# TritonDataCenter/node-zkstream

Measured on AMD Instinct MI355X. Metric: ZK ops/sec (whole node) + p50 get() RTT, 1M-znode synthetic tree, higher is better.
Workload: dtype uint8

## Files before the change

csrc/kernels/frame_scan.hip:

```cpp
#include "zk_frame_scan.h"

namespace zk {

__global__ __launch_bounds__(256) void fs_rows(
    const uint8_t* __restrict__ buf, const int64_t* __restrict__ n_dev,
    int64_t n_cap, const uint16_t* __restrict__ list,
    const uint16_t* __restrict__ pre, const int64_t* __restrict__ rec_meta,
    const int64_t* __restrict__ rec_entry,
    const int64_t* __restrict__ rec_exit,
    const int64_t* __restrict__ base, const int64_t* __restrict__ bsum,
    const int64_t* __restrict__ lastk, int64_t* __restrict__ foff,
    int32_t* __restrict__ flen, int64_t cap, uint64_t* __restrict__ lbw,
    uint64_t* __restrict__ lbw_tail) {
  __shared__ __attribute__((aligned(16))) uint8_t stage[4][FT_STAGE];
  const int lane = threadIdx.x & 63;
  const int wv = __builtin_amdgcn_readfirstlane((int)(threadIdx.x >> 6));
  const int64_t t = (int64_t)blockIdx.x * 4 + wv;
  const int64_t n = stream_len(n_dev, n_cap);
  if (t == 0) {
    if (lane == 0) {
      lbw_tail[LW_MINS] = 0;
      lbw_tail[LW_MINS + 1] = 0;
      lbw_tail[LW_NOSPEC] = 0;
      lbw_tail[LW_GRID + FL_NB] = 0;
    }
    if (lane < LW_END - LW_BIG) lbw_tail[LW_BIG + lane] = 0;
  }
  if (t * FT_S >= n) return;
  if (lane == 0) {
    lbw[2 * t] = 0;
    lbw[2 * t + 1] = 0;
  }
  if (t > *lastk) return;
  const int64_t b = bsum[t / FK_T] + base[t];
  const int64_t m = rec_meta[t];
  const int64_t x = rec_exit[t];
  const int32_t cnt = m_cnt(m);
  auto row = [&](int32_t k, int64_t p, int64_t q) {
    const int64_t idx = b + k;
    if (idx < cap) {
      foff[idx] = p + 4;
      flen[idx] = (int32_t)(q - p - 4);
    }
  };
  if (m_stale(m)) {
    const int32_t c = __builtin_amdgcn_readfirstlane(
        (int32_t)(rec_entry[t] - t * FT_S));
    fr_walk_stale<false>(buf, n, t, c, cnt, x, stage[wv], lane, row);
    return;
  }
  for (int32_t k = lane; k < cnt; k += 64) {
    int64_t p, q;
    fr_bounds(list, pre, t, m, x, k, p, q);
    row(k, p, q);
  }
}

__global__ __launch_bounds__(64) void fs_small(
    const uint8_t* __restrict__ buf, const int64_t* __restrict__ n_dev,
    int64_t n_cap, int64_t maxp, int64_t* __restrict__ foff,
    int32_t* __restrict__ flen, int64_t cap, int64_t* __restrict__ result) {
  __shared__ __attribute__((aligned(16))) uint8_t sb[FT_STAGE];
  const int lane = threadIdx.x;
  const int64_t n = stream_len(n_dev, n_cap);
  fc_stage<FT_S>(buf, n, 0, sb, lane);
  int32_t c = 0, k = 0;
  bool bad = false;
  const int32_t n32 = (int32_t)n;
  while (c + 4 <= n32) {
    const int32_t len = __builtin_amdgcn_readfirstlane(lds_be32(sb, c));
    if (len < 0 || (int64_t)len > maxp) { bad = true; break; }
    if (c + 4 + len > n32) break;
    if (lane == 0 && k < cap) {
      foff[k] = c + 4;
      flen[k] = len;
    }
    ++k;
    c += 4 + len;
  }
  if (lane == 0) {
    result[0] = k;
    result[1] = c;
    result[2] = bad ? 1 : 0;
    result[3] = k > cap ? 1 : 0;
  }
}

constexpr int32_t FS_LONG = 2;
constexpr int32_t FS_DEFER = 1 << 24;

constexpr int32_t FS_WIN_LONG = 1 << 16;

static int fs_window(int32_t window) {
  window &= FS_WIN_LONG - 1;
  return window <= 256 ? 256 : window <= 512 ? 512
       : window <= 1024 ? 1024 : 2048;
}

static int64_t* g_dbg = nullptr;
static int64_t g_dbg_tiles = 0;
static int64_t* fs_dbg_buf(int64_t tiles) {
  static int on = -1;
  if (on < 0) on = getenv("ZKMI_FS_DBG") != nullptr;
  if (!on) return nullptr;
  if (tiles > g_dbg_tiles) {
    if (g_dbg) (void)hipFree(g_dbg);
    if (hipMalloc(&g_dbg, (tiles + FL_DBG_ROWS) * 8 * 8) != hipSuccess)
      return nullptr;
    (void)hipMemset(g_dbg, 0, (tiles + FL_DBG_ROWS) * 8 * 8);
    g_dbg_tiles = tiles;
  }
  return g_dbg;
}

}

extern "C" {

int64_t zk_frame_scan_workspace(int64_t n) {
  return (int64_t)zk::fs_view(nullptr, n).total;
}

int zk_frame_scan(const uint8_t* buf, const int64_t* n_dev, int64_t n_cap,
                  int64_t maxp, uint8_t* ws, int64_t ws_bytes, int64_t* foff,
                  int32_t* flen, int64_t cap, int64_t* result, int32_t window,
                  int32_t clean, int32_t flags, hipStream_t st) {
  using namespace zk;
  const int W = fs_window(window);
  const bool defer = (flags & FS_DEFER) != 0;
  flags &= ~FS_DEFER;
  if (window & FS_WIN_LONG) flags |= FS_LONG;
  if (maxp > FC_MAXP || maxp < 0) return -3;
  const FsWs v = fs_view(ws, n_cap);
  if ((int64_t)v.total > ws_bytes) return -1;
  const int64_t tiles = v.tiles;
  if (defer && n_cap <= FT_S) return -5;
  if (n_cap <= FT_S && !(flags & (1 | 0xFFFF00)) &&
      fs_dbg_buf(tiles) == nullptr) {
    fs_small<<<1, 64, 0, st>>>(buf, n_dev, n_cap, maxp, foff, flen, cap,
                               result);
    ZK_LAUNCH_CHECK();
    return 0;
  }
  if (!clean && hipMemsetAsync(v.lbw, 0, v.lbw_bytes, st) != hipSuccess)
    return -4;
  int64_t* dbg = fs_dbg_buf(tiles);
  int G = ((flags >> 4) & 15) + 1;
  if ((flags & (FS_LONG | 1 | 0xFFFF00)) || W > 512) G = 1;
  G = G >= 8 ? 8 : G >= 4 ? 4 : G >= 2 ? 2 : 1;
  const TileLaunch tl{buf, n_dev, n_cap, maxp, &v, dbg, flags, W, G,
                      (flags & FS_LONG) != 0};
  int rc = G == 1 ? tile_launch(tl, st)
           : W == 256 ? group256_launch(tl, st) : group512_launch(tl, st);
  if (rc) return rc;
  rc = link_launch(buf, n_dev, n_cap, maxp, v, cap, result,
                   dbg ? dbg + 8 * tiles : nullptr, st);
  if (rc || defer) return rc;
  fs_rows<<<(unsigned)((tiles + 3) / 4), 256, 0, st>>>(
      buf, n_dev, n_cap, v.list, v.pre, v.rmeta, v.rent, v.rexit, v.base,
      v.bsum, &v.tail->lastk, foff, flen, cap, v.lbw, (uint64_t*)v.tail);
  ZK_LAUNCH_CHECK();
  return 0;
}

int zk_frame_tiles(const uint8_t* buf, const int64_t* n_dev, int64_t n_cap,
                   uint8_t* ws, int64_t ws_bytes, ZkFrameTiles* out) {
  using namespace zk;
  if (n_cap <= FT_S) return -2;
  const FsWs v = fs_view(ws, n_cap);
  if ((int64_t)v.total > ws_bytes) return -1;
  out->buf = buf;
  out->n_dev = n_dev;
  out->n_cap = n_cap;
  out->list = v.list;
  out->pre = v.pre;
  out->rec_meta = v.rmeta;
  out->rec_entry = v.rent;
  out->rec_exit = v.rexit;
  out->base = v.base;
  out->bsum = v.bsum;
  out->lastk = &v.tail->lastk;
  out->fblk = v.fblk;
  out->lbw = v.lbw;
  out->tiles = v.tiles;
  return 0;
}

int zk_frame_scan_stats(const uint8_t* ws, int64_t n_cap, uint32_t* out4,
                        hipStream_t st) {
  using namespace zk;
  FsTail* t = fs_view(const_cast<uint8_t*>(ws), n_cap).tail;
  const uint64_t* word[4] = {&t->nospec_total, &t->walked, &t->rounds,
                             &t->looked};
  for (int k = 0; k < 4; ++k)
    if (hipMemcpyAsync(out4 + k, word[k], 4, hipMemcpyDeviceToHost, st) !=
        hipSuccess)
      return -1;
  if (hipStreamSynchronize(st) != hipSuccess) return -1;
  if (hipMemsetAsync(t, 0, offsetof(FsTail, mins), st) != hipSuccess)
    return -1;
  return hipStreamSynchronize(st) == hipSuccess ? 0 : -1;
}

int zk_frame_scan_dbg(int64_t* host, int64_t tiles) {
  if (!zk::g_dbg || tiles > zk::g_dbg_tiles + zk::FL_DBG_ROWS) return -1;
  return hipMemcpy(host, zk::g_dbg, tiles * 8 * 8, hipMemcpyDeviceToHost) ==
                 hipSuccess ? 0 : -1;
}

}
```

csrc/kernels/zk_frame_tile.h:

```cpp
#pragma once
#include "zk_frame_scan.h"

namespace zk {

constexpr int FT_BITS = FT_S / 32;
constexpr int FT_XW = 2048 / 32;

ZK_DEV void ft_record(uint16_t* L, int32_t& m, uint32_t& ent, int32_t c,
                      int lane) {
  ent = lane == (m & 63) ? (uint32_t)c : ent;
  ++m;
  if ((m & 63) == 0) L[m - 64 + lane] = (uint16_t)ent;
}

ZK_DEV int32_t ft_starts_below(const uint32_t* sbits, int32_t c, int lane) {
  static_assert(FT_BITS == 2 * 64, "two map words per lane");
  const int32_t cw = c >> 5;
  int32_t below = 0;
#pragma unroll
  for (int h = 0; h < 2; ++h) {
    const int32_t wi = lane + 64 * h;
    const uint32_t wd = sbits[wi];
    below += wi < cw ? __popc(wd)
                     : (wi == cw ? __popc(wd & ((1u << (c & 31)) - 1u)) : 0);
  }
#pragma unroll
  for (int d = 32; d >= 1; d >>= 1) below += __shfl_xor(below, d, 64);
  return below;
}

ZK_DEV int64_t ft_cand(const uint8_t* sb, const uint32_t* sbits, int32_t e,
                       int32_t nrel, int32_t maxp, int64_t send, int64_t n,
                       int64_t ts, int32_t m, int lane) {
  int32_t c = e;
  int32_t hops = 0;
  for (;;) {
    if (c >= FT_S) return (ts + c) | ((int64_t)hops << CX_SHIFT);
    if (ts + c >= n) return FC_LIVE;
    const uint32_t smw = sbits[c >> 5];
    const int32_t lraw = lds_be32(sb, c);
    if ((smw >> (c & 31)) & 1u) {
      if (send & TERM) return (send & TBAD) ? FC_DEAD : FC_LIVE;
      const int32_t below = ft_starts_below(sbits, c, lane);
      return send | ((int64_t)(hops + m - below) << CX_SHIFT);
    }
    if (c + 4 > nrel) return FC_LIVE;
    const int32_t len = __builtin_amdgcn_readfirstlane(lraw);
    if ((uint32_t)len > (uint32_t)maxp) return FC_DEAD;
    const int32_t nx = c + 4 + len;
    if (nx > nrel) return FC_LIVE;
    ++hops;
    c = nx;
  }
}

constexpr int FT_NMAX = 512;
constexpr int FT_SLOTS = 352;
constexpr int32_t FT_LIMIT = FT_S;
enum : uint32_t {
  RK_NODE = 0, RK_EXIT = 1, RK_END = 2, RK_PART = 3, RK_BAD = 4, RK_SHORT = 5
};
ZK_DEV uint32_t rk(uint32_t kind, uint32_t val, uint32_t cnt) {
  return kind << 29 | val << 16 | cnt;
}
ZK_DEV uint32_t rk_kind(uint32_t w) { return w >> 29; }
ZK_DEV uint32_t rk_val(uint32_t w) { return (w >> 16) & 0x1FFF; }
ZK_DEV uint32_t rk_cnt(uint32_t w) { return w & 0xFFFF; }

constexpr int FT_SLOT_B = 704;
constexpr int FT_O_BLK = FT_STAGE;
constexpr int FT_O_BASE = FT_O_BLK + 64 * 8;
constexpr int FT_O_PK = FT_O_BASE + 64 * 2;
constexpr int FT_O_R = FT_O_PK + FT_NMAX * 4;
constexpr int FT_R_B = FT_NMAX * 2 > FT_SLOT_B + FT_XW * 4
                           ? FT_NMAX * 2 : FT_SLOT_B + FT_XW * 4;
constexpr int FT_O_XB = FT_O_R + FT_SLOT_B;
constexpr int FT_LDS = FT_O_R + FT_R_B;
static_assert(FT_SLOT_B >= FT_SLOTS * 2 && FT_SLOT_B >= FT_BITS * 4, "slots");
static_assert(FT_STAGE % 16 == 0 && FT_LDS % 16 == 0, "LDS alignment");

ZK_DEV int32_t be32_of(uint32_t lo, uint32_t hi, int32_t p) {
  return (int32_t)bswap32(__builtin_amdgcn_alignbyte(hi, lo, p & 3));
}

struct FtBlk {
  const uint64_t* mask;
  const uint16_t* base;
};

ZK_DEV bool ft_node(const FtBlk& blk, int32_t q, int32_t& idx) {
  const uint64_t m = blk.mask[q >> 6];
  const int32_t b = blk.base[q >> 6];
  const uint64_t bit = 1ull << (q & 63);
  idx = b + __popcll(m & (bit - 1));
  return (m & bit) != 0;
}

ZK_DEV uint32_t ft_classify(int32_t q, int32_t len, int32_t nrel,
                            int32_t maxp, int32_t minb, uint32_t before) {
  if (q + 4 > nrel) return rk(RK_PART, q, before);
  if ((uint32_t)len > (uint32_t)maxp) return rk(RK_BAD, q, before);
  const int32_t nx = q + 4 + len;
  if (nx > nrel) return rk(RK_PART, q, before);
  if (len < minb) return rk(RK_SHORT, q, before);
  if (nx >= FT_S) return rk(RK_EXIT, q, before + 1);
  return nx == nrel ? rk(RK_END, q, before + 1) : rk(RK_SHORT, q, before);
}

ZK_DEV uint32_t ft_root_at(const uint8_t* sb, const FtBlk& blk,
                           const uint32_t* pk, int32_t e, int32_t nrel,
                           int32_t maxp, int32_t minb) {
  int32_t j;
  if (ft_node(blk, e, j)) return pk[j];
  return ft_classify(e, lds_be32(sb, e), nrel, maxp, minb, 0);
}

ZK_DEV int32_t ft_next(const uint8_t* sb, int32_t p) {
  return p + 4 + lds_be32(sb, p);
}

ZK_DEV int64_t ft_cx(const uint8_t* sb, uint32_t w, int64_t ts) {
  switch (rk_kind(w)) {
    case RK_EXIT:
      return (ts + ft_next(sb, (int32_t)rk_val(w))) |
             ((int64_t)rk_cnt(w) << CX_SHIFT);
    case RK_BAD: return FC_DEAD;
    default: return FC_LIVE;
  }
}

ZK_DEV int64_t ft_send(const uint8_t* sb, uint32_t w, int64_t ts) {
  const int32_t v = (int32_t)rk_val(w);
  switch (rk_kind(w)) {
    case RK_EXIT: return ts + ft_next(sb, v);
    case RK_END: return TERM | (ts + ft_next(sb, v));
    case RK_BAD: return TERM | TBAD | (ts + v);
    default: return TERM | (ts + v);
  }
}

template <int NK>
struct FtNodes {
  int32_t p[NK];
  uint32_t w[NK];
};

template <int NK>
ZK_DEV int ft_build(FtNodes<NK>& me, const uint8_t* sb, const FtBlk& blk,
                    uint32_t* pk, const uint16_t* pos, int32_t N,
                    int32_t nrel, int32_t maxp, int32_t minb, int lane) {
#pragma unroll
  for (int k = 0; k < NK; ++k) {
    const int32_t i = lane + 64 * k;
    const int32_t p = pos[i < N ? i : 0];
// ... 120 lines not shown

template <int W>
ZK_DEV int32_t ft_cands_walk(const uint8_t* sb, const FtBlk& blk,
                             uint32_t* xbits, int32_t nrel, int32_t maxp,
                             int32_t& sx, int lane) {
  uint64_t best = 0;
  for (int r = 0; r < 2; ++r) {
    int32_t want = lane + 64 * r, p = -1;
    for (int b = 0; b < W / 64 && p < 0; ++b) {
      uint64_t m = blk.mask[b];
      const int32_t c = __popcll(m);
      if (want < c) {
        for (int k = 0; k < want; ++k) m &= m - 1;
        p = b * 64 + (int32_t)__builtin_ctzll(m);
      } else {
        want -= c;
      }
    }
    if (!__ballot(p >= 0)) break;
    int32_t c = p, cnt = 0, x = -1;
    bool live = p >= 0;
    while (live) {
      if (c + 4 > nrel) break;
      const int32_t len = lds_be32(sb, c);
      if ((uint32_t)len > (uint32_t)maxp) break;
      const int32_t nx = c + 4 + len;
      if (nx > nrel) break;
      ++cnt;
      if (nx >= FT_S) { x = nx - FT_S; break; }
      c = nx;
    }
    if (x >= 0) {
      if (x < W)
        __hip_atomic_fetch_or(&xbits[x >> 5], 1u << (x & 31),
                              __ATOMIC_RELAXED, __HIP_MEMORY_SCOPE_WAVEFRONT);
      const uint64_t key = (uint64_t)((uint32_t)cnt << 16 |
                                      (uint32_t)(0xFFFF - p)) << 32 |
                           (uint32_t)x;
      best = best > key ? best : key;
    }
  }
#pragma unroll
  for (int s = 32; s >= 1; s >>= 1) {
    const uint64_t o = (uint64_t)__shfl_xor((long long)best, s, 64);
    best = best > o ? best : o;
  }
  if (!best) return -1;
  sx = (int32_t)(uint32_t)best;
  return 0xFFFF - (int32_t)((best >> 32) & 0xFFFF);
}

template <int NK>
ZK_DEV int32_t ft_chain(const FtNodes<NK>& me, const uint8_t* sb,
                        const FtBlk& blk, uint16_t* slot, int32_t e,
                        uint32_t w, int lane) {
  const uint32_t kind = rk_kind(w);
  const int32_t D = (int32_t)rk_cnt(w);
  if (kind == RK_SHORT || kind == RK_BAD || D > FT_SLOTS) return -1;
  if (D == 0) return 0;
  const uint32_t root = w >> 16;
  int32_t hits = 0;
  bool on[NK];
#pragma unroll
  for (int k = 0; k < NK; ++k) {
    const int32_t c = (int32_t)rk_cnt(me.w[k]);
    const int32_t p = me.p[k];
    on[k] = p >= e && (me.w[k] >> 16) == root && c >= 1 && c <= D;
    if (on[k]) slot[D - c] = (uint16_t)p;
    hits += __popcll(__ballot(on[k]));
  }
  __builtin_amdgcn_wave_barrier();
  int32_t want = D;
  if (lane == 0) {
    slot[0] = (uint16_t)e;
    if (kind == RK_EXIT || kind == RK_END) slot[D - 1] = (uint16_t)rk_val(w);
  }
  if (kind == RK_EXIT || kind == RK_END) {
    int32_t j;
    if (!ft_node(blk, (int32_t)rk_val(w), j)) --want;
  }
  __builtin_amdgcn_wave_barrier();
  if (hits == want) return D;
  auto linked = [&]() {
    bool ok = true;
    for (int32_t k = lane; k < D; k += 64) {
      const int32_t p = slot[k];
      const int32_t nx = ft_next(sb, p);
      if (k + 1 < D) {
        ok &= nx == (int32_t)slot[k + 1];
      } else if (kind == RK_PART) {
        ok &= nx == (int32_t)rk_val(w);
      }
    }
    return __ballot(!ok) == 0;
  };
  if (linked()) return D;
  for (int it = 0; it < 8; ++it) {
    int32_t cur[NK];
#pragma unroll
    for (int k = 0; k < NK; ++k)
      cur[k] = on[k] ? (int32_t)slot[D - (int32_t)rk_cnt(me.w[k])] : 0;
    bool wr = false;
#pragma unroll
    for (int k = 0; k < NK; ++k) {
      if (on[k] && me.p[k] < cur[k]) {
        slot[D - (int32_t)rk_cnt(me.w[k])] = (uint16_t)me.p[k];
        wr = true;
      }
    }
    __builtin_amdgcn_wave_barrier();
    if (!__ballot(wr)) break;
  }
  return linked() ? D : -1;
}


struct FtTileRegs {
  uint4 v[FT_S / 16 / 64];
  uint4 pad;
};
ZK_DEV void ft_load(const uint8_t* __restrict__ buf, int64_t n, int64_t ts,
                    int lane, FtTileRegs& r) {
  constexpr int PER = FT_S / 16 / 64;
  r.pad = make_uint4(0, 0, 0, 0);
  if (ts + FT_STAGE <= n) {
#pragma unroll
    for (int j = 0; j < PER; ++j)
      __builtin_memcpy(&r.v[j], buf + ts + 16 * (lane + 64 * j), 16);
    if (lane == 0) __builtin_memcpy(&r.pad, buf + ts + FT_S, 16);
  } else {
#pragma unroll
    for (int j = 0; j < PER; ++j) {
      uint8_t* b = (uint8_t*)&r.v[j];
      const int64_t g = ts + 16 * (lane + 64 * j);
      for (int k = 0; k < 16; ++k) b[k] = g + k < n ? buf[g + k] : 0;
    }
    if (lane == 0) {
      uint8_t* b = (uint8_t*)&r.pad;
      for (int k = 0; k < 16; ++k)
        b[k] = ts + FT_S + k < n ? buf[ts + FT_S + k] : 0;
    }
  }
}
ZK_DEV void ft_store(uint8_t* sb, const FtTileRegs& r, int lane) {
  constexpr int PER = FT_S / 16 / 64;
#pragma unroll
  for (int j = 0; j < PER; ++j) *(uint4*)(sb + 16 * (lane + 64 * j)) = r.v[j];
  if (lane == 0) *(uint4*)(sb + FT_S) = r.pad;
  __builtin_amdgcn_wave_barrier();
}

ZK_DEV int64_t ft_walk(const uint8_t* sb, int32_t c, int32_t nrel,
                       int32_t maxp32, int64_t ts, uint16_t* L, int32_t& mo,
                       int lane) {
  int32_t m = 0, pb = 0;
  uint32_t ent = 0;
  int64_t send;
  c = __builtin_amdgcn_readfirstlane(c);
  nrel = __builtin_amdgcn_readfirstlane(nrel);
  const int32_t lim = min((int32_t)FT_S, nrel);
  if (c >= nrel) {
    send = TERM | (ts + c);
  } else {
    int32_t len = 0, nx = 0, last = 0;
    bool ok = true, fin = false;
    while (!fin) {
      len = __builtin_amdgcn_readfirstlane(lds_be32(sb, c));
      nx = c + 4 + len;
      ok = (uint32_t)len <= (uint32_t)maxp32 && nx <= nrel;
      if (!ok) break;
      ent = lane == (m & 63) ? (uint32_t)c : ent;
      ++m;
      if ((m & 63) == 0) {
        const int32_t q = m - 64 + lane;
        if (q >= pb) L[q] = (uint16_t)ent;
        pb = m;
      }
      if (nx >= lim) break;
      c = nx;
      if (4 + len != last) {
        last = 4 + len;
        continue;
      }
      const int32_t st = last;
      for (;;) {
        const int64_t s64 = (int64_t)c + (int64_t)lane * st;
        const int32_t sp = s64 < lim ? (int32_t)s64 : lim;
        const int32_t lv = sp < lim ? lds_be32(sb, sp) : -1;
        const bool acc = sp < lim && lv == st - 4 && sp + st <= nrel;
        const uint64_t no = ~__ballot(acc);
        const int32_t a = no ? (int32_t)__builtin_ctzll(no) : 64;
        if (a == 0) break;
        const uint64_t end = __ballot(acc && sp + st >= lim);
        const int32_t f = end ? (int32_t)__builtin_ctzll(end) : 64;
        const int32_t r = min(a, f + 1);
        const int32_t q = (m & ~63) + lane;
        if (q >= pb && q < m) L[q] = (uint16_t)ent;
        if (lane < r) L[m + lane] = (uint16_t)sp;
        m += r;
        pb = m;
        nx = c + r * st;
        len = st - 4;
        if (nx >= lim) {
          fin = true;
          break;
        }
        c = nx;
      }
    }
    if (!ok) {
      const bool bad = (c + 4 <= nrel) && ((len < 0) | (len > maxp32));
      send = TERM | (bad ? TBAD : 0) | (ts + c);
    } else if (nx >= FT_S) {
      send = ts + nx;
    } else {
      send = TERM | (ts + nx);
    }
  }
  {
    const int32_t q = (m & ~63) + lane;
    if (q >= pb && q < m) L[q] = (uint16_t)ent;
  }
  mo = m;
  return send;
}

ZK_DEV uint64_t ft_wait_prev(const uint64_t* lbw, int64_t t) {
  uint64_t x;
  int nap = 0;
  const uint64_t t_w = wall_clock64();
  for (;;) {
    x = lb_load(&lbw[2 * (t - 1)]);
    if (x != 0) break;
    if (wall_clock64() - t_w > FT_WAIT_TICKS) break;
    if (nap < 16) __builtin_amdgcn_s_sleep(2);
    else if (nap < 32) __builtin_amdgcn_s_sleep(8);
    else __builtin_amdgcn_s_sleep(32);
    ++nap;
  }
  return x;
}

ZK_DEV int64_t ft_pick(int64_t ts, bool has, int32_t e, int64_t xe,
                       uint32_t we, bool open, uint32_t& wE, bool& known) {
  const uint64_t hm = __ballot(has);
  const uint64_t lm = __ballot(has && xe != FC_DEAD);
  if (lm) {
    const int l = (int)__builtin_ctzll(lm);
    wE = (uint32_t)__builtin_amdgcn_readlane((int)we, l);
    known = !__builtin_amdgcn_readlane((int)open, l);
    return ts + __builtin_amdgcn_readlane(e, l);
  }
  return hm ? ts + __builtin_amdgcn_readlane(e, (int)__builtin_ctzll(hm)) : -1;
}

template <typename At>
ZK_DEV void ft_survivor_bits(uint32_t* sbits, int32_t m, int lane, At at) {
  for (int k = lane; k < FT_SLOT_B / 4; k += 64) sbits[k] = 0u;
  __builtin_amdgcn_wave_barrier();
  for (int i = lane; i < m; i += 64) {
    const uint32_t q = at(i);
    __hip_atomic_fetch_or(&sbits[q >> 5], 1u << (q & 31), __ATOMIC_RELAXED,
                          __HIP_MEMORY_SCOPE_WAVEFRONT);
  }
  __builtin_amdgcn_wave_barrier();
}

struct FtCtx {
  const uint8_t* buf;
  uint16_t* list;
  uint16_t* pre;
  int64_t* sx;
  uint64_t* lbw;
  int64_t* rec_entry;
  int64_t* rec_exit;
  int64_t* rec_meta;
  int32_t* rcount;
  int64_t* dbg;
  int64_t* cx;
  uint64_t* stats;
  uint8_t* sb;
  FtBlk blk;
  uint32_t* pk;
  uint16_t* pos;
  uint16_t* slot;
  uint32_t* sbits;
  uint32_t* xbits;
  int64_t n, t, ts, tend, t_0, t_s, t_d;
  int32_t nrel, maxp32, minb, N, misspec;
  bool nospec;
  int lane;
};

ZK_DEV void ft_join(const FtCtx& C, int64_t E, int32_t m, int64_t send,
                    FcWalk& wk) {
  const int lane = C.lane;
  const uint8_t* sb = C.sb;
  const int64_t n = C.n, ts = C.ts;
  const int32_t nrel = C.nrel, maxp32 = C.maxp32;
  int64_t c = E;
  uint16_t* P = C.pre + C.t * FT_LMAX;
  int32_t np = 0;
  uint32_t ent = 0;
  for (;;) {
    if (c >= C.tend) { wk.exit = c; break; }
    if (c >= n) { wk.exit = n; break; }
    const int32_t crel = (int32_t)(c - ts);
    const uint32_t smw = C.sbits[crel >> 5];
    const int32_t lraw = lds_be32(sb, crel);
    if ((smw >> (crel & 31)) & 1u) {
      wk.js = ft_starts_below(C.sbits, crel, lane);
      break;
    }
    const int32_t len = __builtin_amdgcn_readfirstlane(lraw);
    const int32_t nx = crel + 4 + len;
    if ((uint32_t)len > (uint32_t)maxp32 || nx > nrel) {
      wk.exit = c;
      wk.term = true;
      wk.bad = (crel + 4 <= nrel) && ((len < 0) | (len > maxp32));
      break;
    }
    ft_record(P, np, ent, crel, lane);
    c = ts + nx;
  }
  if (lane < (np & 63)) P[(np & ~63) + lane] = (uint16_t)ent;
  wk.np = np;
  wk.cnt = np;
  if (wk.js >= 0) {
    wk.cnt = np + (m - wk.js);
    fc_join_end(wk, send, n);
  }
}

ZK_DEV void ft_put_record(const FtCtx& C, int64_t t, int64_t send, int32_t m,
                          int64_t entry, const FcWalk& wk) {
  if (C.lane != 0) return;
  C.sx[t] = send;
  C.rcount[t] = m;
  C.rec_entry[t] = entry;
  C.rec_exit[t] = wk.exit;
  C.rec_meta[t] = fc_meta(wk);
}

ZK_DEV void ft_put_mapped(const FtCtx& C, int64_t send, int32_t m,
                          int64_t entry, const FcWalk& wk, int64_t t_1,
                          int64_t t_2, int64_t t_f, int rounds, bool done) {
  ft_put_record(C, C.t, send, m, entry, wk);
  if (C.lane == 0 && C.dbg) {
    int64_t* d = C.dbg + 8 * C.t;
    d[0] = C.t_0;
    d[1] = t_1;
    d[2] = t_2;
    d[3] = wall_clock64();
    d[4] = C.t_d;
    d[5] = (int64_t)C.N | (int64_t)rounds << 16 | (int64_t)done << 24;
    d[6] = C.t_s;
    d[7] = t_f;
  }
}

template <int W, bool LONG, int NK>
ZK_DEV int64_t fs_tile_rest(const FtCtx& cx_, bool mapped) {
  const FtCtx& C = cx_;
  const int lane = C.lane;
  const uint8_t* sb = C.sb;
  const int64_t n = C.n, t = C.t, ts = C.ts, tend = C.tend;
  const int32_t nrel = C.nrel, maxp32 = C.maxp32, minb = C.minb;
  constexpr int XW = W / 32;
  FtNodes<NK> me;
  int rounds = 0;
  if (mapped)
    rounds = ft_build<NK>(me, sb, C.blk, C.pk, C.pos, C.N, nrel, maxp32, minb,
                          lane);
  for (int k = lane; k < FT_R_B / 4; k += 64) C.sbits[k] = 0u;
  __builtin_amdgcn_wave_barrier();
  const int64_t t_f = C.dbg ? wall_clock64() : 0;

  int32_t px = -1, sp = -1;
  {
    int32_t x = -1;
    sp = mapped ? ft_cands<W, LONG, NK>(me, sb, C.xbits, x)
                : ft_cands_walk<W>(sb, C.blk, C.xbits, nrel, maxp32, x, lane);
    if (sp >= 0 && x >= 0 && x < (LONG ? FT_S - 1 : W)) px = x;
  }
  __builtin_amdgcn_wave_barrier();
  uint64_t word = (uint64_t)1 << 63;
  if (px >= 0) word |= (uint64_t)(px + 1);
  {
    uint32_t xw = lane < XW ? C.xbits[lane] : 0u;
    if (px >= 0 && px < W && lane == (px >> 5)) xw &= ~(1u << (px & 31));
    uint64_t any = __ballot(xw != 0);
    int nsl = 1;
    if (px < 0 && any) {
      const int wl = (int)__builtin_ctzll(any);
      const uint32_t bits = (uint32_t)__builtin_amdgcn_readlane((int)xw, wl);
      const int x0 = wl * 32 + (int)__builtin_ctz(bits);
      word |= (uint64_t)(x0 + 1);
      if (lane == wl) xw &= ~(1u << (x0 & 31));
      any = __ballot(xw != 0);
    }
    while (any && nsl < 5) {
      const int wl = (int)__builtin_ctzll(any);
      uint32_t bits = (uint32_t)__builtin_amdgcn_readlane((int)xw, wl);
      while (bits && nsl < 5) {
        const int bit = (int)__builtin_ctz(bits);
        bits &= bits - 1;
        word |= (uint64_t)(wl * 32 + bit + 1) << (12 * nsl);
        ++nsl;
      }
      any &= any - 1;
    }
  }
  if (lane == 0) lb_store(&C.lbw[2 * t], word);
  const int64_t t_1 = C.dbg ? wall_clock64() : 0;

  int64_t E = 0;
  bool none = false;
  uint32_t wE = 0;
  bool wE_ok = false;
  if (t > 0 && C.nospec) {
    none = true;
    if (lane < 5) C.cx[5 * t + lane] = FC_DEAD;
  } else if (t > 0) {
    const uint64_t x = ft_wait_prev(C.lbw, t);
    const int32_t v = lane < 5 ? (int32_t)((x >> (12 * lane)) & 0xFFF) : 0;
    const bool has = v != 0 && ts + (v - 1) < n;
    const int32_t e = v - 1;
    uint32_t we = 0;
    if (has && mapped) we = ft_root_at(sb, C.blk, C.pk, e, nrel, maxp32, minb);
    const bool open = has && (!mapped || rk_kind(we) == RK_SHORT);
    int64_t xe = has && !open ? ft_cx(sb, we, ts) : FC_DEAD;
    for (uint64_t um = __ballot(open); um; um &= um - 1) {
      const int l = (int)__builtin_ctzll(um);
      const int32_t el = __builtin_amdgcn_readlane(e, l);
      const int64_t r = ft_cand(sb, C.sbits, el, nrel, maxp32, -1, n, ts, 0,
                                lane);
      if (lane == l) xe = r;
    }
    if (lane < 5) C.cx[5 * t + lane] = xe;
    E = ft_pick(ts, has, e, xe, we, open, wE, wE_ok);
    wE_ok = wE_ok && mapped;
    if (C.misspec > 0 && t % C.misspec == 1 && E >= 0 && E + 1 < n) {
      ++E;
      wE_ok = false;
    }
    none = E < 0;
  }
  const int64_t t_2 = C.dbg ? wall_clock64() : 0;

  uint16_t* L = C.list + t * FT_LMAX;
  FcWalk wk{E, 0, 0, -1, false, false};
  int64_t send = -1;
  int32_t m = 0;
  bool done = false;
  const int32_t erel = (int32_t)(E - ts);
  if (!none && erel >= nrel) {
    send = TERM | E;
    fc_join_end(wk, send, n);
    done = true;
  } else if (!none && mapped) {
    const uint32_t we = wE_ok ? wE
                              : ft_root_at(sb, C.blk, C.pk, erel, nrel, maxp32,
                                           minb);
    const int32_t D = ft_chain<NK>(me, sb, C.blk, C.slot, erel, we, lane);
    if (D >= 0) {
      for (int32_t k = lane; k < D; k += 64) L[k] = C.slot[k];
      m = D;
      send = ft_send(sb, we, ts);
      wk.cnt = D;
      wk.js = D > 0 ? 0 : -1;
      fc_join_end(wk, send, n);
      done = true;
    }
  }
  if (!done) {
    if (sp >= 0 && mapped) {
      const uint32_t ws = ft_root_at(sb, C.blk, C.pk, sp, nrel, maxp32, minb);
      const int32_t D = ft_chain<NK>(me, sb, C.blk, C.slot, sp, ws, lane);
      if (D > 0) {
        for (int32_t k = lane; k < D; k += 64) L[k] = C.slot[k];
        m = D;
        send = ft_send(sb, ws, ts);
      }
    } else if (sp >= 0) {
      __builtin_amdgcn_wave_barrier();
      send = ft_walk(sb, sp, nrel, maxp32, ts, L, m, lane);
      if (m == 0) send = -1;
    }
    __builtin_amdgcn_wave_barrier();
    ft_survivor_bits(C.sbits, m, lane, [&](int i) { return (uint32_t)L[i]; });
    if (!none) {
      ft_join(C, E, m, send, wk);
    } else {
      if (m > 0) fc_join_end(wk, send, n);
      if (lane == 0) fc_stat(C.stats, 1, 1), fc_stat(C.stats, LW_NOSPEC, 1);
    }
  }
  ft_put_mapped(C, send, m, none ? -1 : E, wk, t_1, t_2, t_f, rounds, done);
  return send;
}


ZK_DEV int64_t ft_cx_of(int64_t send, int32_t m) {
  if (!(send & TERM)) return send | ((int64_t)m << CX_SHIFT);
  return (send & TBAD) ? FC_DEAD : FC_LIVE;
}

template <int SVN>
ZK_DEV int32_t ft_sv_at(const uint32_t (&sv)[SVN], int32_t q) {
  uint32_t v = 0;
#pragma unroll
  for (int i = 0; i < SVN; ++i)
    if (i == (q >> 6)) v = sv[i];
  return __builtin_amdgcn_readlane((int)v, q & 63);
}

template <int W, int G>
ZK_DEV void ft_group_tail(const FtCtx& C, int64_t send0, bool alive,
                          FtTileRegs& nxt) {
  const int lane = C.lane;
  uint8_t* sb = C.sb;
  const int64_t n = C.n, t0 = C.t;
  const int32_t maxp32 = C.maxp32;
  const int64_t ntiles = (n + FT_S - 1) / FT_S;
  int64_t send = send0;
  int32_t kdone = 1;
  for (int k = 1; k < G; ++k) {
    const int64_t tk = t0 + k;
    if (tk >= ntiles) break;
    const int64_t tsk = tk * FT_S;
    const int64_t c = send;
    const bool live = alive && !(send & TERM) && c >= tsk &&
                      c < tsk + FT_S;
    if (!live) break;
    int64_t* const dk = C.dbg ? C.dbg + 8 * tk : nullptr;
    const int64_t k_0 = dk ? wall_clock64() : 0;
    ft_store(sb, nxt, lane);
    const int64_t k_1 = dk ? wall_clock64() : 0;
    if (k + 1 < G && tk + 1 < ntiles) ft_load(C.buf, n, tsk + FT_S, lane, nxt);
    int32_t m;
    const int32_t nrelk = (int32_t)min(n - tsk, (int64_t)1 << 30);
    send = ft_walk(sb, (int32_t)(c - tsk), nrelk, maxp32, tsk,
                   C.list + tk * FT_LMAX, m, lane);
    const int64_t k_2 = dk ? wall_clock64() : 0;
    FcWalk wk{c, m, 0, m > 0 ? 0 : -1, false, false};
    fc_join_end(wk, send, n);
    ft_put_record(C, tk, send, m, c, wk);
    if (lane == 0) {
      lb_store(&C.lbw[2 * (tk - 1)],
               (uint64_t)1 << 63 | (uint64_t)(c - tsk + 1));
      C.cx[5 * tk] = ft_cx_of(send, m);
      if (dk) {
        dk[0] = k_0;
        dk[1] = k_1;
        dk[2] = k_2;
        dk[3] = wall_clock64();
        dk[5] = (int64_t)m;
      }
    }
    if (lane >= 1 && lane < 5) C.cx[5 * tk + lane] = FC_DEAD;
    kdone = k + 1;
  }
  for (int k = kdone; k < G; ++k) {
    const int64_t tk = t0 + k;
    if (tk >= ntiles) break;
    if (lane == 0) lb_store(&C.lbw[2 * (tk - 1)], (uint64_t)1 << 63);
    ft_put_record(C, tk, -1, 0, -1, FcWalk{-1, 0, 0, -1, false, false});
    if (lane < 5) C.cx[5 * tk + lane] = FC_DEAD;
  }
  const int64_t tl = min(t0 + G, ntiles) - 1;
  {
    uint64_t word = (uint64_t)1 << 63;
    const int64_t tle = (tl + 1) * FT_S;
    if (kdone == (int32_t)(tl - t0 + 1) && alive && !(send & TERM) &&
        send >= tle && send < tle + W)
      word |= (uint64_t)(send - tle + 1);
    if (lane == 0) lb_store(&C.lbw[2 * tl], word);
  }
}

template <int W, int NK, int G>
ZK_DEV void fs_group_rest(const FtCtx& cx_) {
  static_assert(G > 1 && W <= 512, "groups: small windows");
  constexpr int WJ = W / 64;
  const FtCtx& C = cx_;
  const int lane = C.lane;
  uint8_t* sb = C.sb;
  const int64_t n = C.n, t0 = C.t, ts = C.ts;
  const int32_t nrel = C.nrel, maxp32 = C.maxp32, minb = C.minb;
  const int64_t ntiles = (n + FT_S - 1) / FT_S;
  FtNodes<NK> me;
  const int rounds = ft_build<NK>(me, sb, C.blk, C.pk, C.pos, C.N, nrel,
                                  maxp32, minb, lane);
  for (int k = lane; k < FT_R_B / 4; k += 64) C.sbits[k] = 0u;
  __builtin_amdgcn_wave_barrier();
  const int64_t t_f = C.dbg ? wall_clock64() : 0;

  int32_t x = -1;
  const int32_t sp = ft_cands<W, false, NK>(me, sb, C.xbits, x);
  uint32_t rw[WJ];
  int64_t rx[WJ];
#pragma unroll
  for (int j = 0; j < WJ; ++j) {
    const int32_t e = lane + 64 * j;
    rw[j] = e < nrel ? ft_root_at(sb, C.blk, C.pk, e, nrel, maxp32, minb)
                     : rk(RK_END, 0, 0);
    rx[j] = e < nrel ? ft_cx(sb, rw[j], ts) : FC_LIVE;
  }
  int32_t m0 = 0;
  int64_t send0 = -1;
  uint32_t ws = 0;
  uint16_t* L0 = C.list + t0 * FT_LMAX;
  if (sp >= 0) {
    ws = ft_root_at(sb, C.blk, C.pk, sp, nrel, maxp32, minb);
    const int32_t D = ft_chain<NK>(me, sb, C.blk, C.slot, sp, ws, lane);
    if (D >= 0) {
      for (int32_t k = lane; k < D; k += 64) L0[k] = C.slot[k];
      m0 = D;
      send0 = ft_send(sb, ws, ts);
    } else {
      __builtin_amdgcn_wave_barrier();
      send0 = ft_walk(sb, sp, nrel, maxp32, ts, L0, m0, lane);
      for (int32_t k = lane; k < m0; k += 64) C.slot[k] = L0[k];
      ws = 0;
    }
  }
  constexpr int SVN = (FT_SLOTS + 63) / 64;
  __builtin_amdgcn_wave_barrier();
  uint32_t sv[SVN];
#pragma unroll
  for (int i = 0; i < SVN; ++i)
    sv[i] = lane + 64 * i < m0 ? C.slot[lane + 64 * i] : 0u;
  const int64_t t_1 = C.dbg ? wall_clock64() : 0;

  FtTileRegs nxt;
  if (G > 1 && t0 + 1 < ntiles) ft_load(C.buf, n, ts + FT_S, lane, nxt);
  ft_group_tail<W, G>(C, send0, sp >= 0, nxt);

  int64_t E = 0;
  bool none = false;
  uint32_t wE = 0;
  bool known = false;
  bool staged = false;
  auto restage = [&]() {
    if (staged) return;
    FtTileRegs r;
    ft_load(C.buf, n, ts, lane, r);
    ft_store(sb, r, lane);
    ft_survivor_bits(C.sbits, m0, lane, [&](int i) {
      uint32_t v = 0;
#pragma unroll
      for (int k = 0; k < SVN; ++k)
        if (k == (i >> 6)) v = sv[k];
      return v;
    });
    staged = true;
  };
  if (t0 > 0) {
    const uint64_t xw = ft_wait_prev(C.lbw, t0);
    const int32_t v = lane < 5 ? (int32_t)((xw >> (12 * lane)) & 0xFFF) : 0;
    const bool has = v != 0 && ts + (v - 1) < n;
    const int32_t e = v - 1;
    uint32_t we = 0;
    int64_t xe = FC_DEAD;
    bool open = false;
    for (int s = 0; s < 5; ++s) {
      const int32_t es = __builtin_amdgcn_readlane(e, s);
      if (!__builtin_amdgcn_readlane((int)has, s)) continue;
      if (es >= W) {
        if (lane == s) open = true;
        continue;
      }
      const int jj = es >> 6, ll = es & 63;
      uint32_t wv = 0;
      int64_t xv = 0;
#pragma unroll
      for (int j = 0; j < WJ; ++j)
        if (j == jj) { wv = rw[j]; xv = rx[j]; }
      const uint32_t wsv = (uint32_t)__builtin_amdgcn_readlane((int)wv, ll);
      const int64_t xsv = (int64_t)(
          (uint64_t)(uint32_t)__builtin_amdgcn_readlane((int)(uint32_t)xv,
                                                         ll) |
          (uint64_t)(uint32_t)__builtin_amdgcn_readlane(
              (int)(uint32_t)((uint64_t)xv >> 32), ll) << 32);
      if (lane == s) {
        we = wsv;
        xe = xsv;
        open = rk_kind(wsv) == RK_SHORT;
      }
    }
    if (__ballot(open)) {
      restage();
      for (uint64_t um = __ballot(open); um; um &= um - 1) {
        const int l = (int)__builtin_ctzll(um);
        const int32_t el = __builtin_amdgcn_readlane(e, l);
        const int64_t r = ft_cand(sb, C.sbits, el, nrel, maxp32, send0, n,
                                  ts, m0, lane);
        if (lane == l) xe = r;
      }
    }
    if (lane < 5) C.cx[5 * t0 + lane] = xe;
    E = ft_pick(ts, has, e, xe, we, open, wE, known);
    none = E < 0;
  } else {
    wE = rw[0];
    wE = (uint32_t)__builtin_amdgcn_readlane((int)wE, 0);
    known = true;
  }
  const int64_t t_2 = C.dbg ? wall_clock64() : 0;

  FcWalk wk{E, 0, 0, -1, false, false};
  const int32_t erel = (int32_t)(E - ts);
  bool done = false;
  if (!none && erel >= nrel) {
    fc_join_end(wk, TERM | E, n);
    done = true;
  } else if (!none && known && ws != 0 && (wE >> 16) == (ws >> 16) &&
             (int32_t)rk_cnt(wE) <= m0 && rk_cnt(wE) > 0 &&
             ft_sv_at<SVN>(sv, m0 - (int32_t)rk_cnt(wE)) == erel) {
    wk.js = m0 - (int32_t)rk_cnt(wE);
    wk.cnt = (int32_t)rk_cnt(wE);
    fc_join_end(wk, send0, n);
    done = true;
  }
  if (!done && !none) {
    restage();
    ft_join(C, E, m0, send0, wk);
  } else if (none) {
    if (m0 > 0) fc_join_end(wk, send0, n);
    if (lane == 0) fc_stat(C.stats, 1, 1), fc_stat(C.stats, LW_NOSPEC, 1);
  }
  ft_put_mapped(C, send0, m0, none ? -1 : E, wk, t_1, t_2, t_f, rounds, done);
}

template <int W, bool LONG, int G>
__global__ __launch_bounds__(256) void fs_tile(
    const uint8_t* __restrict__ buf, const int64_t* __restrict__ n_dev,
    int64_t n_cap, int64_t maxp, uint16_t* __restrict__ list,
    uint16_t* __restrict__ pre, int64_t* __restrict__ sx, uint64_t* lbw,
    int64_t* __restrict__ rec_entry, int64_t* __restrict__ rec_exit,
    int64_t* __restrict__ rec_meta, int32_t* __restrict__ rcount,
    int64_t ntiles_cap, int64_t* __restrict__ dbg, int32_t minb,
    int32_t tflags, int64_t* __restrict__ cx) {
  static_assert(W % 64 == 0 && W <= 2048, "window");
  extern __shared__ __attribute__((aligned(16))) uint8_t smem_all[];
  const int wv = __builtin_amdgcn_readfirstlane((int)(threadIdx.x >> 6));
  uint8_t* smem = smem_all + wv * FT_LDS;
  FtCtx C;
  C.sb = smem;
  uint64_t* bmask = (uint64_t*)(smem + FT_O_BLK);
  uint16_t* bbase = (uint16_t*)(smem + FT_O_BASE);
  C.blk.mask = bmask;
  C.blk.base = bbase;
  C.pk = (uint32_t*)(smem + FT_O_PK);
  C.pos = (uint16_t*)(smem + FT_O_R);
  C.slot = (uint16_t*)(smem + FT_O_R);
  C.sbits = (uint32_t*)(smem + FT_O_R);
  C.xbits = (uint32_t*)(smem + FT_O_XB);
  const int lane = threadIdx.x & 63;
  const int64_t n = stream_len(n_dev, n_cap);
  const int64_t ntiles = (n + FT_S - 1) / FT_S;
  const int64_t t = ((int64_t)blockIdx.x * (blockDim.x >> 6) + wv) * G;
  if (t >= ntiles) return;
  C.t_0 = dbg ? wall_clock64() : 0;
  const int64_t ts = t * FT_S;
  const int64_t tend = ts + FT_S;
  const int32_t nrel = (int32_t)min(n - ts, (int64_t)1 << 30);
  const int32_t maxp32 = (int32_t)maxp;
  uint8_t* sb = C.sb;

  {
    FtTileRegs r;
    ft_load(buf, n, ts, lane, r);
    ft_store(sb, r, lane);
  }
  C.t_s = dbg ? (__builtin_amdgcn_s_waitcnt(0), wall_clock64()) : 0;

  int32_t N;
  {
    const int32_t P0 = lane * 64;
    uint32_t d[17];
    {
      const int r = (lane >> 2) & 3;
      uint4 x0 = *(const uint4*)(sb + P0 + 16 * (r & 3));
      uint4 x1 = *(const uint4*)(sb + P0 + 16 * ((1 + r) & 3));
      uint4 x2 = *(const uint4*)(sb + P0 + 16 * ((2 + r) & 3));
      uint4 x3 = *(const uint4*)(sb + P0 + 16 * ((3 + r) & 3));
      const uint32_t pad = *(const uint32_t*)(sb + FT_S);
      auto sel = [](bool c, uint4 a, uint4 b) {
        return make_uint4(c ? a.x : b.x, c ? a.y : b.y, c ? a.z : b.z,
                          c ? a.w : b.w);
      };
      {
        const bool c = r & 1;
        const uint4 y0 = sel(c, x3, x0), y1 = sel(c, x0, x1),
                    y2 = sel(c, x1, x2), y3 = sel(c, x2, x3);
        x0 = y0; x1 = y1; x2 = y2; x3 = y3;
      }
      {
        const bool c = r & 2;
        const uint4 y0 = sel(c, x2, x0), y1 = sel(c, x3, x1),
                    y2 = sel(c, x0, x2), y3 = sel(c, x1, x3);
        x0 = y0; x1 = y1; x2 = y2; x3 = y3;
      }
      d[0] = x0.x; d[1] = x0.y; d[2] = x0.z; d[3] = x0.w;
      d[4] = x1.x; d[5] = x1.y; d[6] = x1.z; d[7] = x1.w;
      d[8] = x2.x; d[9] = x2.y; d[10] = x2.z; d[11] = x2.w;
      d[12] = x3.x; d[13] = x3.y; d[14] = x3.z; d[15] = x3.w;
      const uint32_t nx = (uint32_t)__shfl_down((int)d[0], 1, 64);
      d[16] = lane == 63 ? pad : nx;
    }
    const uint32_t lim = P0 < W ? (uint32_t)(maxp32 - minb + 1)
                         : LONG ? (uint32_t)(FT_LIMIT - minb)
                                : (uint32_t)(W - 3 - minb);
    uint32_t lo = 0, hi = 0;
#pragma unroll
    for (int j = 0; j < 32; ++j) {
      const uint32_t v = (uint32_t)be32_of(d[j >> 2], d[(j >> 2) + 1], j);
      lo |= ((v - (uint32_t)minb) < lim ? 1u : 0u) << j;
    }
#pragma unroll
    for (int j = 32; j < 64; ++j) {
      const uint32_t v = (uint32_t)be32_of(d[j >> 2], d[(j >> 2) + 1], j);
      hi |= ((v - (uint32_t)minb) < lim ? 1u : 0u) << (j - 32);
    }
    uint64_t mask = (uint64_t)hi << 32 | lo;
    const int32_t room = nrel - 4 - P0;
    if (room < 63) mask = room < 0 ? 0 : mask & ((2ull << room) - 1);
    const uint32_t c = (uint32_t)__popcll(mask);
    uint32_t incl = c;
#pragma unroll
    for (int s = 1; s < 64; s <<= 1) {
      const uint32_t y = __shfl_up(incl, s, 64);
      if (lane >= s) incl += y;
    }
    N = __builtin_amdgcn_readlane((int)incl, 63);
    const uint32_t base = incl - c;
    bmask[lane] = mask;
    bbase[lane] = (uint16_t)base;
    if (N <= FT_NMAX) {
      uint32_t k = base;
      uint64_t m = mask;
      while (m) {
        C.pos[k++] = (uint16_t)(P0 + __builtin_ctzll(m));
        m &= m - 1;
      }
    }
  }
  __builtin_amdgcn_wave_barrier();
  C.t_d = dbg ? wall_clock64() : 0;
  C.buf = buf; C.list = list; C.pre = pre; C.sx = sx; C.lbw = lbw;
  C.rec_entry = rec_entry; C.rec_exit = rec_exit; C.rec_meta = rec_meta;
  C.rcount = rcount; C.dbg = dbg; C.cx = cx;
  C.stats = &lbw[2 * ntiles_cap];
  C.n = n; C.t = t; C.ts = ts; C.tend = tend;
  C.nrel = nrel; C.maxp32 = maxp32; C.minb = minb; C.N = N;
  C.nospec = tflags & 1;
  C.misspec = tflags >> 8;
  C.lane = lane;
  static_assert(FT_NMAX == 512, "node buckets");
  if constexpr (G > 1) {
    static_assert(!LONG, "groups: frames within the window");
    if (N <= 128) fs_group_rest<W, 2, G>(C);
    else if (N <= 256) fs_group_rest<W, 4, G>(C);
    else if (N <= FT_NMAX) fs_group_rest<W, 8, G>(C);
    else {
      const int64_t s0 = fs_tile_rest<W, LONG, 1>(C, false);
      FtTileRegs nxt;
      if (t + 1 < (n + FT_S - 1) / FT_S) ft_load(buf, n, ts + FT_S, lane, nxt);
      ft_group_tail<W, G>(C, s0, s0 >= 0, nxt);
    }
  } else {
    if (N <= 128) fs_tile_rest<W, LONG, 2>(C, true);
    else if (N <= 256) fs_tile_rest<W, LONG, 4>(C, true);
    else if (N <= FT_NMAX) fs_tile_rest<W, LONG, 8>(C, true);
    else fs_tile_rest<W, LONG, 1>(C, false);
  }
}



template <int W, bool LONG, int G>
int fs_tile_launch(const TileLaunch& l, hipStream_t st) {
  const FsWs& w = *l.ws;
  const int64_t waves = (w.tiles + G - 1) / G;
  const unsigned blocks = (unsigned)((waves + FS_TPB - 1) / FS_TPB);
  fs_tile<W, LONG, G><<<blocks, 64 * FS_TPB, FT_LDS * FS_TPB, st>>>(
      l.buf, l.n_dev, l.n_cap, l.maxp, w.list, w.pre, w.sx, w.lbw, w.rent,
      w.rexit, w.rmeta, w.rcnt, w.tiles, l.dbg, FS_MINB, l.tflags, w.cx);
  ZK_LAUNCH_CHECK();
  return 0;
}

template <int W>
int fs_group_launch(const TileLaunch& l, hipStream_t st) {
  switch (l.G) {
    case 8: return fs_tile_launch<W, false, 8>(l, st);
    case 4: return fs_tile_launch<W, false, 4>(l, st);
    case 2: return fs_tile_launch<W, false, 2>(l, st);
    default: return -1;
  }
}

}
```

Baseline: 2.188 billion.

## Skip tiles in group tail by gathering fixed-stride frame runs in bulk

When the frames ending a tile form a run of equal length, the group tail now checks the whole strided run with one gathered global load per lane. It then writes records, list entries and link words for every tile the run covers, so those tiles skip the serial per-tile walk. The register survivor vector becomes a 16-bit LDS array, which saves registers. Group mode is also allowed when the debug, nospec and misspec flags are set, and the commit adds nospec and misspec test paths. The risk lies in correctness on edge cases such as runs crossing tiles and partial final frames.

After: 2.312 billion, median of 6. 1.06x the previous value.

```diff
diff --git a/csrc/kernels/frame_scan.hip b/csrc/kernels/frame_scan.hip
--- a/csrc/kernels/frame_scan.hip
+++ b/csrc/kernels/frame_scan.hip
@@ -146,7 +146,7 @@
     return -4;
   int64_t* dbg = fs_dbg_buf(tiles);
   int G = ((flags >> 4) & 15) + 1;
-  if ((flags & (FS_LONG | 1 | 0xFFFF00)) || W > 512) G = 1;
+  if ((flags & FS_LONG) || W > 512) G = 1;
   G = G >= 8 ? 8 : G >= 4 ? 4 : G >= 2 ? 2 : 1;
   const TileLaunch tl{buf, n_dev, n_cap, maxp, &v, dbg, flags, W, G,
                       (flags & FS_LONG) != 0};
diff --git a/csrc/kernels/zk_frame_tile.h b/csrc/kernels/zk_frame_tile.h
--- a/csrc/kernels/zk_frame_tile.h
+++ b/csrc/kernels/zk_frame_tile.h
@@ -1,5 +1,6 @@
 #pragma once
 #include "zk_frame_scan.h"
+#include "zk_run_span.h"
 
 namespace zk {
 
@@ -426,17 +427,19 @@
 
 ZK_DEV int64_t ft_walk(const uint8_t* sb, int32_t c, int32_t nrel,
                        int32_t maxp32, int64_t ts, uint16_t* L, int32_t& mo,
-                       int lane) {
+                       int lane, int32_t& last, bool& run) {
   int32_t m = 0, pb = 0;
   uint32_t ent = 0;
   int64_t send;
   c = __builtin_amdgcn_readfirstlane(c);
   nrel = __builtin_amdgcn_readfirstlane(nrel);
+  last = __builtin_amdgcn_readfirstlane(last);
+  run = false;
   const int32_t lim = min((int32_t)FT_S, nrel);
   if (c >= nrel) {
     send = TERM | (ts + c);
   } else {
-    int32_t len = 0, nx = 0, last = 0;
+    int32_t len = 0, nx = 0;
     bool ok = true, fin = false;
     while (!fin) {
       len = __builtin_amdgcn_readfirstlane(lds_be32(sb, c));
@@ -450,12 +453,18 @@
         if (q >= pb) L[q] = (uint16_t)ent;
         pb = m;
       }
-      if (nx >= lim) break;
+      if (nx >= lim) {
+        run = 4 + len == last;
+        last = 4 + len;
+        break;
+      }
       c = nx;
       if (4 + len != last) {
         last = 4 + len;
+        run = false;
         continue;
       }
+      run = true;
       const int32_t st = last;
       for (;;) {
         const int64_t s64 = (int64_t)c + (int64_t)lane * st;
@@ -606,14 +615,17 @@
   }
 }
 
-ZK_DEV void ft_put_record(const FtCtx& C, int64_t t, int64_t send, int32_t m,
-                          int64_t entry, const FcWalk& wk) {
-  if (C.lane != 0) return;
+ZK_DEV void ft_put_record_lane(const FtCtx& C, int64_t t, int64_t send,
+                               int32_t m, int64_t entry, const FcWalk& wk) {
   C.sx[t] = send;
   C.rcount[t] = m;
   C.rec_entry[t] = entry;
   C.rec_exit[t] = wk.exit;
   C.rec_meta[t] = fc_meta(wk);
+}
+ZK_DEV void ft_put_record(const FtCtx& C, int64_t t, int64_t send, int32_t m,
+                          int64_t entry, const FcWalk& wk) {
+  if (C.lane == 0) ft_put_record_lane(C, t, send, m, entry, wk);
 }
 
 ZK_DEV void ft_put_mapped(const FtCtx& C, int64_t send, int32_t m,
@@ -758,7 +770,9 @@
       }
     } else if (sp >= 0) {
       __builtin_amdgcn_wave_barrier();
-      send = ft_walk(sb, sp, nrel, maxp32, ts, L, m, lane);
+      int32_t last = 0;
+      bool run;
+      send = ft_walk(sb, sp, nrel, maxp32, ts, L, m, lane, last, run);
       if (m == 0) send = -1;
     }
     __builtin_amdgcn_wave_barrier();
@@ -780,26 +794,127 @@
   return (send & TBAD) ? FC_DEAD : FC_LIVE;
 }
 
-template <int SVN>
-ZK_DEV int32_t ft_sv_at(const uint32_t (&sv)[SVN], int32_t q) {
-  uint32_t v = 0;
-#pragma unroll
-  for (int i = 0; i < SVN; ++i)
-    if (i == (q >> 6)) v = sv[i];
-  return __builtin_amdgcn_readlane((int)v, q & 63);
+constexpr int FT_NGI = 4;
+static_assert(RUN_TILE == FT_S, "zk_run_span.h: the tile");
+struct FtGather {
+  uint32_t w[FT_NGI];
+  int32_t crel, S, room, want, nrel;
+  int64_t g_0;
+};
+ZK_DEV FtGather ft_gather_issue(const FtCtx& C, int64_t c, int32_t S,
+                                int64_t tk, int64_t gend) {
+  FtGather g;
+  const int64_t tsk = tk * FT_S;
+  g.crel = __builtin_amdgcn_readfirstlane((int32_t)(c - tsk));
+  g.S = __builtin_amdgcn_readfirstlane(S);
+  g.g_0 = C.dbg ? wall_clock64() : 0;
+  g.room = (int32_t)(gend - tk);
+  g.nrel = (int32_t)min(C.n - tsk, (int64_t)1 << 30);
+  g.want = run_want(g.crel, g.S, g.room * FT_S, 64 * FT_NGI);
+  const uint8_t* tb = C.buf + tsk;
+#pragma unroll
+  for (int i = 0; i < FT_NGI; ++i) {
+    const int32_t j = C.lane + 64 * i;
+    const int32_t prel = g.crel + j * g.S;
+    g.w[i] = 0;
+    if (j < g.want && run_word_in(prel, g.nrel))
+      __builtin_memcpy(&g.w[i], tb + prel, 4);
+  }
+  return g;
+}
+ZK_DEV int32_t ft_gather_take(const FtCtx& C, const FtGather& g, int64_t tk,
+                              int64_t& send, bool& full) {
+  const int lane = C.lane;
+  const int64_t n = C.n, tsk = tk * FT_S;
+  const int32_t crel = g.crel, S = g.S, want = g.want, room = g.room;
+  const uint32_t(&w)[FT_NGI] = g.w;
+  const int64_t g_0 = g.g_0;
+  const int64_t g_1 =
+      C.dbg ? (__builtin_amdgcn_s_waitcnt(0), wall_clock64()) : 0;
+  int32_t a = 0;
+  bool open = true;
+#pragma unroll
+  for (int i = 0; i < FT_NGI; ++i) {
+    const int32_t j = lane + 64 * i;
+    const int32_t prel = crel + j * S;
+    const bool acc = j < want && run_word_in(prel, g.nrel) &&
+                     run_accept((int32_t)bswap32(w[i]), S, prel, g.nrel,
+                                C.maxp32);
+    const uint64_t no = ~__ballot(acc);
+    const int32_t ai = no ? (int32_t)__builtin_ctzll(no) : 64;
+    a += open ? ai : 0;
+    open = open && ai == 64;
+  }
+  full = a == 64 * FT_NGI;
+  const int32_t cov = min(run_tiles_covered(crel, S, a), room);
+  if (cov == 0) return 0;
+  const int64_t g_2 = C.dbg ? wall_clock64() : 0;
+  int32_t rfirst = 0;
+  if (lane < cov) {
+    const RunTile r = run_tile(crel, S, a, lane);
+    rfirst = r.first;
+    const int64_t tq = tk + lane;
+    const int64_t entry = tsk + r.entry, exit = tsk + r.exit;
+    FcWalk wk{entry, r.count, 0, r.count > 0 ? 0 : -1, false, false};
+    fc_join_end(wk, exit, n);
+    ft_put_record_lane(C, tq, exit, r.count, entry, wk);
+    lb_store(&C.lbw[2 * (tq - 1)],
+             (uint64_t)1 << 63 | (uint64_t)(entry - tq * FT_S + 1));
+    C.cx[5 * tq] = ft_cx_of(exit, r.count);
+#pragma unroll
+    for (int s = 1; s < 5; ++s) C.cx[5 * tq + s] = FC_DEAD;
+    if (C.dbg) {
+      int64_t* const dk = C.dbg + 8 * tq;
+      dk[0] = g_0;
+      dk[1] = g_1;
+      dk[2] = g_2;
+      dk[3] = wall_clock64();
+      dk[5] = (int64_t)r.count;
+    }
+  }
+#pragma unroll
+  for (int i = 0; i < FT_NGI; ++i) {
+    const int32_t j = lane + 64 * i;
+    const int32_t prel = crel + j * S;
+    const int32_t q = prel >> 12;
+    const int32_t first = __shfl(rfirst, q & 63, 64);
+    if (j < a && q < cov) {
+      C.list[(tk + q) * FT_LMAX + (j - first)] = (uint16_t)(prel & (FT_S - 1));
+    }
+  }
+  send = tsk + run_tile(crel, S, a, cov - 1).exit;
+  return cov;
 }
 
 template <int W, int G>
 ZK_DEV void ft_group_tail(const FtCtx& C, int64_t send0, bool alive,
-                          FtTileRegs& nxt) {
+                          FtTileRegs& nxt, int32_t last, bool run) {
   const int lane = C.lane;
   uint8_t* sb = C.sb;
   const int64_t n = C.n, t0 = C.t;
   const int32_t maxp32 = C.maxp32;
   const int64_t ntiles = (n + FT_S - 1) / FT_S;
+  const int64_t gend = min(t0 + G, ntiles);
   int64_t send = send0;
   int32_t kdone = 1;
-  for (int k = 1; k < G; ++k) {
+  int k = 1;
+  if (W <= 256 && run && last >= 16 && last <= FT_S && t0 + 1 < ntiles &&
+      alive && !(send & TERM)) {
+    bool full = true, first = true;
+    while (full && k < G && t0 + k < ntiles && send >= (t0 + k) * FT_S &&
+           send < (t0 + k + 1) * FT_S) {
+      const FtGather g = ft_gather_issue(C, send, last, t0 + k, gend);
+      if (first) ft_store(sb, nxt, lane);
+      first = false;
+      const int32_t cov = ft_gather_take(C, g, t0 + k, send, full);
+      if (cov == 0) break;
+      k += cov;
+    }
+    kdone = k;
+    if (k < G && t0 + k < ntiles)
+      ft_load(C.buf, n, (t0 + k) * FT_S, lane, nxt);
+  }
+  for (; k < G; ++k) {
     const int64_t tk = t0 + k;
     if (tk >= ntiles) break;
     const int64_t tsk = tk * FT_S;
@@ -815,7 +930,7 @@
     int32_t m;
     const int32_t nrelk = (int32_t)min(n - tsk, (int64_t)1 << 30);
     send = ft_walk(sb, (int32_t)(c - tsk), nrelk, maxp32, tsk,
-                   C.list + tk * FT_LMAX, m, lane);
+                   C.list + tk * FT_LMAX, m, lane, last, run);
     const int64_t k_2 = dk ? wall_clock64() : 0;
     FcWalk wk{c, m, 0, m > 0 ? 0 : -1, false, false};
     fc_join_end(wk, send, n);
@@ -894,22 +1009,31 @@
       send0 = ft_send(sb, ws, ts);
     } else {
       __builtin_amdgcn_wave_barrier();
-      send0 = ft_walk(sb, sp, nrel, maxp32, ts, L0, m0, lane);
+      int32_t last = 0;
+      bool run;
+      send0 = ft_walk(sb, sp, nrel, maxp32, ts, L0, m0, lane, last, run);
       for (int32_t k = lane; k < m0; k += 64) C.slot[k] = L0[k];
       ws = 0;
     }
   }
-  constexpr int SVN = (FT_SLOTS + 63) / 64;
+  static_assert(FT_SLOTS * 2 <= FT_NMAX * 4, "the starts fit the node words");
   __builtin_amdgcn_wave_barrier();
-  uint32_t sv[SVN];
-#pragma unroll
-  for (int i = 0; i < SVN; ++i)
-    sv[i] = lane + 64 * i < m0 ? C.slot[lane + 64 * i] : 0u;
+  uint16_t* const sv = (uint16_t*)C.pk;
+  for (int32_t k = lane; k < m0; k += 64) sv[k] = C.slot[k];
+  __builtin_amdgcn_wave_barrier();
+  int32_t last0 = 0;
+  bool run0 = false;
+  if (m0 >= 1 && send0 >= 0 && !(send0 & TERM)) {
+    const int32_t a = __builtin_amdgcn_readfirstlane(sv[m0 - 1]);
+    const int32_t b = __builtin_amdgcn_readfirstlane(sv[m0 >= 2 ? m0 - 2 : 0]);
+    last0 = (int32_t)(send0 - ts) - a;
+    run0 = m0 >= 2 && a - b == last0;
+  }
   const int64_t t_1 = C.dbg ? wall_clock64() : 0;
 
   FtTileRegs nxt;
   if (G > 1 && t0 + 1 < ntiles) ft_load(C.buf, n, ts + FT_S, lane, nxt);
-  ft_group_tail<W, G>(C, send0, sp >= 0, nxt);
+  ft_group_tail<W, G>(C, send0, sp >= 0, nxt, last0, run0);
 
   int64_t E = 0;
   bool none = false;
@@ -921,16 +1045,14 @@
     FtTileRegs r;
     ft_load(C.buf, n, ts, lane, r);
     ft_store(sb, r, lane);
-    ft_survivor_bits(C.sbits, m0, lane, [&](int i) {
-      uint32_t v = 0;
-#pragma unroll
-      for (int k = 0; k < SVN; ++k)
-        if (k == (i >> 6)) v = sv[k];
-      return v;
-    });
+    ft_survivor_bits(C.sbits, m0, lane,
+                     [&](int i) { return (uint32_t)sv[i]; });
     staged = true;
   };
-  if (t0 > 0) {
+  if (t0 > 0 && C.nospec) {
+    none = true;
+    if (lane < 5) C.cx[5 * t0 + lane] = FC_DEAD;
+  } else if (t0 > 0) {
     const uint64_t xw = ft_wait_prev(C.lbw, t0);
     const int32_t v = lane < 5 ? (int32_t)((xw >> (12 * lane)) & 0xFFF) : 0;
     const bool has = v != 0 && ts + (v - 1) < n;
@@ -975,6 +1097,10 @@
     }
     if (lane < 5) C.cx[5 * t0 + lane] = xe;
     E = ft_pick(ts, has, e, xe, we, open, wE, known);
+    if (C.misspec > 0 && (t0 / G) % C.misspec == 1 && E >= 0 && E + 1 < n) {
+      ++E;
+      known = false;
+    }
     none = E < 0;
   } else {
     wE = rw[0];
@@ -991,7 +1117,8 @@
     done = true;
   } else if (!none && known && ws != 0 && (wE >> 16) == (ws >> 16) &&
              (int32_t)rk_cnt(wE) <= m0 && rk_cnt(wE) > 0 &&
-             ft_sv_at<SVN>(sv, m0 - (int32_t)rk_cnt(wE)) == erel) {
+             __builtin_amdgcn_readfirstlane(
+                 (int32_t)sv[m0 - (int32_t)rk_cnt(wE)]) == erel) {
     wk.js = m0 - (int32_t)rk_cnt(wE);
     wk.cnt = (int32_t)rk_cnt(wE);
     fc_join_end(wk, send0, n);
@@ -1142,7 +1269,7 @@
       const int64_t s0 = fs_tile_rest<W, LONG, 1>(C, false);
       FtTileRegs nxt;
       if (t + 1 < (n + FT_S - 1) / FT_S) ft_load(buf, n, ts + FT_S, lane, nxt);
-      ft_group_tail<W, G>(C, s0, s0 >= 0, nxt);
+      ft_group_tail<W, G>(C, s0, s0 >= 0, nxt, 0, false);
     }
   } else {
     if (N <= 128) fs_tile_rest<W, LONG, 2>(C, true);
diff --git a/csrc/kernels/zk_run_span.h b/csrc/kernels/zk_run_span.h
--- /dev/null
+++ b/csrc/kernels/zk_run_span.h
@@ -0,0 +1,49 @@
+#pragma once
+#include <stdint.h>
+
+#include "zk_wire.h"
+
+namespace zk {
+
+constexpr int32_t RUN_TILE = 4096;
+
+
+ZK_HD bool run_word_in(int32_t p, int32_t nrel) {
+  return p >= 0 && p + 4 <= nrel;
+}
+
+ZK_HD bool run_accept(int32_t len, int32_t S, int32_t p, int32_t nrel,
+                      int32_t maxp) {
+  return len == S - 4 && p + S <= nrel && (uint32_t)len <= (uint32_t)maxp;
+}
+
+ZK_HD int32_t run_want(int32_t crel, int32_t S, int32_t gerel, int32_t cap) {
+  const int32_t w = (gerel - crel + S - 1) / S;
+  return w < cap ? w : cap;
+}
+
+ZK_HD int32_t run_frames_before(int32_t S, int32_t count, int32_t xrel) {
+  if (xrel <= 0) return 0;
+  const int32_t k = (xrel + S - 1) / S;
+  return k < count ? k : count;
+}
+
+ZK_HD int32_t run_tiles_covered(int32_t crel, int32_t S, int32_t count) {
+  return (int32_t)(((int64_t)crel + (int64_t)count * S) / RUN_TILE);
+}
+
+struct RunTile {
+  int32_t first, count;
+  int32_t entry, exit;
+};
+ZK_HD RunTile run_tile(int32_t crel, int32_t S, int32_t count, int32_t q) {
+  RunTile r;
+  r.first = run_frames_before(S, count, q * RUN_TILE - crel);
+  const int32_t next = run_frames_before(S, count, (q + 1) * RUN_TILE - crel);
+  r.count = next - r.first;
+  r.entry = crel + r.first * S;
+  r.exit = crel + next * S;
+  return r;
+}
+
+}
```
